# mkocabas/EpipolarPose

Measured on NVIDIA H100. Metric: multi-view samples/sec (4-view 256x256, bs32), higher is better.
Workload: dtype f16x3 (fp32 operands split into two fp16 planes, 3-pass error-compensated wgmma f16, f32 accumulate: fp32-grade results)

## Files before the change

epipolarpose_b200/_lib.py:

```python
import ctypes
import os

HERE = os.path.dirname(os.path.abspath(__file__))
LIB_PATH = os.environ.get("EPB_LIB_PATH") or os.path.join(HERE, "libepb.so")

EPB_MAX_TAPS = 64

c_int, c_i64, c_f, c_d, c_p = (ctypes.c_int, ctypes.c_int64, ctypes.c_float,
                               ctypes.c_double, ctypes.c_void_p)


class ConvGeom(ctypes.Structure):
    _fields_ = [("N", c_int), ("Hi", c_int), ("Wi", c_int), ("Cin", c_int),
                ("Ho", c_int), ("Wo", c_int), ("Cout", c_int),
                ("Hp", c_int), ("Wp", c_int),
                ("os", c_int), ("ph", c_int), ("pw", c_int), ("is_", c_int),
                ("T", c_int),
                ("dh", c_int * EPB_MAX_TAPS), ("dw", c_int * EPB_MAX_TAPS),
                ("wt", c_int * EPB_MAX_TAPS), ("Tw", c_int),
                ("in_relu", c_int), ("accumulate", c_int), ("precision", c_int)]


_PROTOS = {
    "epb_version": (c_int, []),
# ... 16 lines not shown
    "epb_bn_bwd_apply": (c_int, [c_p, c_p, c_p, c_p, c_p, c_p, c_p, c_p, c_int, c_p, c_i64, c_int, c_p, c_p, c_p, c_p]),
    "epb_add_masked": (c_int, [c_p, c_p, c_p, c_p, c_i64, c_p]),
    "epb_avgpool": (c_int, [c_p, c_p, c_int, c_int, c_int, c_p]),
    "epb_avgpool_bwd": (c_int, [c_p, c_p, c_int, c_int, c_int, c_int, c_p]),
    "epb_colsum": (c_int, [c_p, c_i64, c_int, c_p, c_p]),
    "epb_softargmax_fwd": (c_int, [c_p, c_int, c_int, c_int, c_int, c_int, c_int, c_p, c_p, c_p]),
    "epb_softargmax_bwd": (c_int, [c_p, c_int, c_int, c_int, c_int, c_int, c_int, c_p, c_p, c_p, c_p, c_p]),
    "epb_jointloss_fwd_bwd": (c_int, [c_p, c_p, c_p, c_int, c_int, c_int, c_f, c_p, c_p, c_p]),
    "epb_heatmap_joint_loss": (c_int, [c_p, c_p, c_p, c_int, c_int, c_f, c_p, c_p, c_p, c_int, c_int, c_f, c_f,
                                       c_p, c_p, c_p, c_p]),
    "epb_argmax2d": (c_int, [c_p, c_int, c_int, c_int, c_p, c_p, c_p, c_p]),
    "epb_final_preds": (c_int, [c_p, c_int, c_int, c_int, c_int, c_p, c_p, c_int, c_p, c_p, c_p]),
    "epb_patch_to_image": (c_int, [c_p, c_p, c_int, c_int, c_d, c_d, c_d, c_p, c_p]),
    "epb_triangulate": (c_int, [c_p, c_p, c_int, c_p, c_p, c_int, c_int, c_int, c_d, c_p, c_p, c_p]),
    "epb_triangulate_nview": (c_int, [c_p, c_int, c_p, c_int, c_int, c_int, c_p, c_p, c_p]),
    "epb_relative_pose": (c_int, [c_p, c_int, c_p, c_p, c_int, c_int, c_d, c_p, c_p, c_p, c_p, c_p, c_p,
                                  c_p]),
    "epb_project_labels": (c_int, [c_p, c_p, c_p, c_int, c_int, c_d, c_d, c_d, c_p, c_p, c_p]),
    "epb_h36m_eval": (c_int, [c_p, c_p, c_p, c_int, c_int, c_int, ctypes.c_uint32, c_d, c_p, c_p, c_p, c_p, c_p]),
    "epb_add3": (c_int, [c_p, c_p, c_p, c_p, c_i64, c_p]),
    "epb_mask_scale": (c_int, [c_p, c_p, c_f, c_p, c_i64, c_p]),
    "epb_patch_sample": (c_int, [c_p, c_p, c_p, c_p, c_p, c_p, c_p, c_int, c_int, c_int, c_p, c_p, c_p]),
    "epb_patch_sample_occ": (c_int, [c_p] * 7 + [c_int, c_int, c_int] + [c_p] * 5 + [c_p]),
    "epb_patch_joints": (c_int, [c_p, c_p, c_p, c_int, c_int, c_d, c_d, c_d, c_int, c_p, c_p]),
    "epb_bn_finalize_scale": (c_int, [c_p, c_i64, c_int, c_p, c_p, c_f, c_f] + [c_p] * 12),
    "epb_softargmax_bwd_split": (c_int, [c_p] + [c_int] * 5 + [c_p] * 7),
    "epb_act_scale": (c_int, [c_p, c_p, c_p, c_i64, c_int, c_p, c_p, c_p, c_p, c_p, c_p]),
    "epb_bn_act_split": (c_int, [c_p] * 8 + [c_int, c_i64, c_int, c_p, c_p, c_p, c_p]),
    "epb_bn_relu_maxpool_split": (c_int, [c_p] * 6 + [c_int] * 4 + [c_p]),
    "epb_im2col_split": (c_int, [c_p] * 3 + [c_int] * 11 + [c_p]),
    "epb_split16": (c_int, [c_p, ctypes.c_longlong, c_p, c_p, c_p, c_p]),
    "epb_split16_batch": (c_int, [c_p, c_int, ctypes.c_longlong, c_p, c_p]),
    "epb_conv16_fprop": (c_int, [ctypes.POINTER(ConvGeom)] + [c_p] * 8),
    "epb_conv16_wgrad": (c_int, [ctypes.POINTER(ConvGeom)] + [c_p] * 6 + [ctypes.c_longlong, c_p]),
    "epb_bn_bwd_reduce_mx": (c_int, [c_p] * 7 + [c_int, c_i64, c_int, c_p, c_p, c_p]),
    "epb_bn_bwd_apply_split": (c_int, [c_p] * 8 + [c_int, c_p, c_p, c_i64, c_int] + [c_p] * 6),
    "epb_bn_bwd_split": (c_int, [c_p] * 9 + [c_int, c_i64, c_int] + [c_p] * 6),
    "epb_avgpool_split": (c_int, [c_p, c_p, c_p, c_int, c_int, c_int, c_p]),
    "epb_sumsq": (c_int, [c_p, c_i64, c_p, c_p]),
    "epb_clip_scale": (c_int, [c_p, c_i64, c_p, c_d, c_p]),
    "epb_adam_step": (c_int, [c_p, c_p, c_p, c_p, c_i64, c_f, c_f, c_f, c_f, c_f, c_int, c_f, c_p]),
    "epb_sgd_step": (c_int, [c_p, c_p, c_p, c_i64, c_f, c_f, c_f, c_int, c_int, c_f, c_p]),
    "epb_adam_step_dev": (c_int, [c_p, c_p, c_p, c_p, c_i64, c_p, c_p, c_p]),
    "epb_sgd_step_dev": (c_int, [c_p, c_p, c_p, c_i64, c_p, c_p, c_p]),
}

EXPORTS = tuple(_PROTOS)


class EpbError(RuntimeError):
    pass


_lib = None


def lib():
    global _lib
    if _lib is None:
        if not os.path.exists(LIB_PATH):
            raise EpbError("libepb.so not built (%s); run `python -c 'import __graft_entry__ as g; "
                           "g.build()'`. There is no CPU fallback." % LIB_PATH)
        L = ctypes.CDLL(LIB_PATH)
        for name, (res, args) in _PROTOS.items():
            fn = getattr(L, name)
            fn.restype = res
            fn.argtypes = args
        _lib = L
    return _lib


def check(rc):
    if rc != 0:
        raise EpbError("libepb call failed (%d): %s" % (rc, lib().epb_last_error().decode()))


def call(name, *args):
    check(getattr(lib(), name)(*args))
```

epipolarpose_b200/csrc/conv16.cu:

```cuda
#include "split16_common.cuh"

namespace {

constexpr int BM = 128;
constexpr int kThreads16 = 384;
constexpr int kConsumers = 256;
constexpr int kStageBudget = 200 * 1024;
constexpr int kBoxBytes = 16 * 128;

struct Plan16 {
  epb_phase_grid grid;
  int Cout;
  int Wv, Hv;
  int T, CB;
  int n_tiles;
  int accumulate;
  int m_fastest;
  int koff[EPB_MAX_TAPS];
};

struct Maps16 {
  CUtensorMap a[4];
  CUtensorMap w;
  CUtensorMap out;
};

template <int BN>
struct Cfg16 {
  static constexpr int A_PLANE = BM * 128;
  static constexpr int B_PLANE = BN * 128;
  static constexpr int A_BYTES = 2 * A_PLANE;
  static constexpr int B_BYTES = 2 * B_PLANE;
  static constexpr int STAGE = A_BYTES + B_BYTES;
  static constexpr int S_ = kStageBudget / STAGE;
  static constexpr int S = S_ > 6 ? 6 : S_;
  static constexpr int BOX_BYTES = (kConsumers / 32) * kBoxBytes;
  static constexpr int STAT_BYTES = (kConsumers / 32) * 2 * BN * 4;
  static constexpr int SMEM =
      S * STAGE + BOX_BYTES + 1024  + 256  + STAT_BYTES;
  static_assert(SMEM <= 227 * 1024, "shared memory budget");
  static_assert(S >= 2, "ring too shallow");
};

template <int BN>
__global__ void __launch_bounds__(kThreads16, 1)
conv16_kernel(const __grid_constant__ Plan16 P, const __grid_constant__ Maps16 maps,
              const float* __restrict__ in_sc, const float* __restrict__ w_sc,
              const float* __restrict__ bias, double* __restrict__ stats) {
  using C = Cfg16<BN>;
  const epb_phase_grid& G = P.grid;
  constexpr int BOXES = C::S * C::STAGE;
  constexpr int CTRL = BOXES + C::BOX_BYTES;
  extern __shared__ uint8_t smem_raw[];
  tc::Ring<C::S, C::STAGE> ring(smem_raw, 0, CTRL, CTRL + 64);
  float* sstat = reinterpret_cast<float*>(ring.sm + CTRL + 256);

  const int warp = threadIdx.x >> 5, lane = threadIdx.x & 31;
  const int KB = P.T * P.CB;
  const int total_tiles = G.tiles * P.n_tiles;
  auto nt_of = [&](int tile) { return P.m_fastest ? tile / G.tiles : tile % P.n_tiles; };
  auto mt_of = [&](int tile) { return P.m_fastest ? tile % G.tiles : tile / P.n_tiles; };

  if (threadIdx.x == 0) ring.init(1, kConsumers / 32);
  __syncthreads();

  if (warp < 4) {
    if (warp == 0 && lane == 0) {
      for (int v = 0; v < 4; ++v) tc::tma_prefetch_desc(&maps.a[v]);
      tc::tma_prefetch_desc(&maps.w);
      tc::tma_prefetch_desc(&maps.out);
      for (int tile = blockIdx.x; tile < total_tiles; tile += gridDim.x) {
        const int nt = nt_of(tile);
        int w0, h0, n0;
        G.tile_origin(mt_of(tile), w0, h0, n0);
        int t = 0, cb = 0;
        for (int kb = 0; kb < KB; ++kb) {
          tc::mbar_wait(ring.empty(ring.stage), ring.phase ^ 1);
          const uint32_t fb = ring.full(ring.stage);
          tc::mbar_arrive_expect_tx(fb, C::STAGE);
          const uint32_t a_dst = ring.stage_addr(ring.stage);
          const CUtensorMap* am = &maps.a[G.map[t]];
          const int cx = cb * 64, wx = w0 + G.dwq[t], hx = h0 + G.dhq[t];
          tc::tma_load_5d(a_dst, am, fb, cx, wx, hx, n0, 0);
          tc::tma_load_5d(a_dst + C::A_PLANE, am, fb, cx, wx, hx, n0, 1);
          const uint32_t b_dst = a_dst + C::A_BYTES;
          const int kx = P.koff[t] + cx, rx = nt * BN;
          tc::tma_load_3d(b_dst, &maps.w, fb, kx, rx, 0);
          tc::tma_load_3d(b_dst + C::B_PLANE, &maps.w, fb, kx, rx, 1);
          if (++cb == P.CB) { cb = 0; ++t; }
          ring.advance();
        }
      }
    }
    return;
  }

  const int wgc = (warp >> 2) - 1;
  const int ct = threadIdx.x - 128;
  float* wstat = sstat + (ct >> 5) * 2 * BN;
  const int lc = (lane & 3) * 2;
  const int rb = wgc * 64 + (warp & 3) * 16;
  const int ra = rb + (lane >> 2);
  uint8_t* box = ring.sm + BOXES + (ct >> 5) * kBoxBytes;
  const uint32_t box_addr = tc::smem_u32(box);
  auto chunk = [&](int jj) { return ((2 * jj + ((lane & 3) >> 1)) ^ (lane >> 2)) * 16 + (lane & 1) * 8; };
  const float alpha = in_sc[1] * w_sc[1];
  const int twh = G.tw * G.th;
  if (stats) {
    for (int c = ct; c < (kConsumers / 32) * 2 * BN; c += kConsumers) sstat[c] = 0.f;
    tc::named_sync(1, kConsumers);
  }

  float acc[BN / 2];
  int nt_prev = -1;
  for (int tile = blockIdx.x; tile < total_tiles; tile += gridDim.x) {
    const int nt = nt_of(tile);
    if (stats && nt_prev >= 0 && nt != nt_prev)
      tc::stats_flush<BN, kConsumers / 32>(sstat, ct, nt_prev, P.Cout, stats);
    nt_prev = nt;
#pragma unroll
    for (int i = 0; i < BN / 2; ++i) acc[i] = 0.f;
    for (int kb = 0; kb < KB; ++kb)
      ring.consume(acc, [&](uint32_t st) {
        const uint32_t a_hi = st + wgc * 64 * 128, b_hi = st + C::A_BYTES;
#pragma unroll
        for (int kk = 0; kk < 4; ++kk)
          tc::mma3_f16<0, 0>(acc, tc::desc_kmajor_sw128(a_hi + kk * 32),
                             tc::desc_kmajor_sw128(a_hi + C::A_PLANE + kk * 32),
                             tc::desc_kmajor_sw128(b_hi + kk * 32),
                             tc::desc_kmajor_sw128(b_hi + C::B_PLANE + kk * 32));
      });
    ring.drain(acc);

    int w0, h0, n0;
    G.tile_origin(mt_of(tile), w0, h0, n0);
    bool srow[2];
#pragma unroll
    for (int h = 0; h < 2; ++h) {
      const int r = ra + 8 * h;
      const int w = w0 + r % G.tw, hh = h0 + (r / G.tw) % G.th, n = n0 + r / twh;
      srow[h] = w < G.Wp && hh < G.Hp && n < G.N;
    }
    const int bx = w0 + rb % G.tw, by = h0 + (rb / G.tw) % G.th, bz = n0 + rb / twh;
    const bool band = bx < P.Wv && by < P.Hv && bz < G.N;
#pragma unroll
    for (int q = 0; q < BN / 32; ++q) {
      if (lane == 0) tc::tma_store_wait_read<0>();
      __syncwarp();
#pragma unroll
      float v[4][2][2];
#pragma unroll
      for (int jj = 0; jj < 4; ++jj) {
        const int col = nt * BN + 32 * q + 8 * jj + lc;
        float2 b = make_float2(0.f, 0.f);
        if (bias && col < P.Cout) b = *reinterpret_cast<const float2*>(bias + col);
#pragma unroll
        for (int h = 0; h < 2; ++h) {
          v[jj][h][0] = acc[16 * q + 4 * jj + 2 * h] * alpha + b.x;
          v[jj][h][1] = acc[16 * q + 4 * jj + 2 * h + 1] * alpha + b.y;
          *reinterpret_cast<float2*>(box + 128 * ((lane >> 2) + 8 * h) + chunk(jj)) =
              make_float2(v[jj][h][0], v[jj][h][1]);
        }
      }
      tc::fence_proxy_async();
      __syncwarp();
      const int c0 = nt * BN + 32 * q;
      if (lane == 0 && band && c0 < P.Cout) {
        if (P.accumulate) tc::tma_reduce_add_4d(&maps.out, box_addr, c0, bx, by, bz);
        else tc::tma_store_4d(&maps.out, box_addr, c0, bx, by, bz);
        tc::tma_store_commit();
      }
      if (stats) {
#pragma unroll
        for (int jj = 0; jj < 4; ++jj) tc::stats_add<BN>(wstat, 32 * q + 8 * jj + lc, v[jj], srow);
      }
    }
  }
  if (stats && nt_prev >= 0) tc::stats_flush<BN, kConsumers / 32>(sstat, ct, nt_prev, P.Cout, stats);
  if (lane == 0) tc::tma_store_wait<0>();
}

}

extern "C" __attribute__((visibility("default"))) int epb_conv16_fprop(
    const epb_conv_geom* g, const epb_half* in, const float* in_sc, const epb_half* w,
    const float* w_sc, const float* bias, float* out, double* stats, epb_stream_t stream) {
  int rc = epb_conv_geom_check(g);
  if (rc) return rc;
  EPB_CHECK_ARG(in && in_sc && w && w_sc && out);
  EPB_CHECK_ARG(g->Cin % 64 == 0 && g->Cout % 4 == 0 && g->Cout >= 4);
  EPB_CHECK_ARG(g->is == 1 || g->is == 2);
  EPB_CHECK_ARG(!(stats && g->accumulate));
  EPB_CHECK_ARG((reinterpret_cast<uintptr_t>(in) & 127) == 0 && (reinterpret_cast<uintptr_t>(w) & 15) == 0);
  EPB_CHECK_ARG((reinterpret_cast<uintptr_t>(out) & 15) == 0 && (reinterpret_cast<uintptr_t>(bias) & 7) == 0);
  Plan16 P;
  Maps16 maps;
  memset(&maps, 0, sizeof(maps));
  bool dense;
  rc = epb_plan_phase_grid(g, in, BM, P.grid, maps.a, dense);
  if (rc) return rc;
  const int64_t Ho = dense ? 1 : g->Ho, Wo = dense ? P.grid.Wp : g->Wo, os = g->os;
  const int64_t ph = dense ? 0 : g->ph, pw = dense ? 0 : g->pw;
  P.Cout = g->Cout;
  P.Wv = dense ? P.grid.Wp : (g->Wo - g->pw + g->os - 1) / g->os;
  P.Hv = dense ? 1 : (g->Ho - g->ph + g->os - 1) / g->os;
  {
    const int bw = P.grid.tw < 16 ? P.grid.tw : 16;
    const int bh = P.grid.th < 16 / bw ? P.grid.th : 16 / bw;
    const int64_t C4 = (int64_t)g->Cout * 4;
    const cuuint64_t dims[4] = {(cuuint64_t)g->Cout, (cuuint64_t)P.Wv, (cuuint64_t)P.Hv,
                                (cuuint64_t)P.grid.N};
    const cuuint64_t strides[3] = {(cuuint64_t)(os * C4), (cuuint64_t)(os * Wo * C4),
                                   (cuuint64_t)(Ho * Wo * C4)};
    const cuuint32_t box[4] = {32, (cuuint32_t)bw, (cuuint32_t)bh, (cuuint32_t)(16 / (bw * bh))};
    rc = epb_encode_map(&maps.out, CU_TENSOR_MAP_DATA_TYPE_FLOAT32, 4, out + (ph * Wo + pw) * g->Cout,
                        dims, strides, box, CU_TENSOR_MAP_L2_PROMOTION_NONE, "output");
    if (rc) return rc;
  }
  P.T = g->T; P.CB = g->Cin / 64; P.accumulate = g->accumulate;
  for (int t = 0; t < g->T; ++t) P.koff[t] = g->wt[t] * g->Cin;
  P.m_fastest = stats != nullptr;
  const int bn = g->Cout <= 64 ? 64 : 128;
  P.n_tiles = (g->Cout + bn - 1) / bn;
  const int64_t K = (int64_t)g->Tw * g->Cin;
  const cuuint64_t dims[3] = {(cuuint64_t)K, (cuuint64_t)g->Cout, 2};
  const cuuint64_t strides[2] = {(cuuint64_t)K * 2, (cuuint64_t)K * 2 * g->Cout};
  const cuuint32_t box[3] = {64, (cuuint32_t)bn, 1};
  rc = epb_encode_map(&maps.w, CU_TENSOR_MAP_DATA_TYPE_FLOAT16, 3, w, dims, strides, box,
                      CU_TENSOR_MAP_L2_PROMOTION_L2_256B, "weights");
  if (rc) return rc;
  const int64_t tiles = (int64_t)P.grid.tiles * P.n_tiles;
  const unsigned grid = (unsigned)(tiles < kNumSMs ? tiles : kNumSMs);
  cudaStream_t st = as_stream(stream);
  if (bn == 64)
    return tc::launch<conv16_kernel<64>>(grid, kThreads16, Cfg16<64>::SMEM, st, P, maps, in_sc,
                                         w_sc, bias, stats);
  return tc::launch<conv16_kernel<128>>(grid, kThreads16, Cfg16<128>::SMEM, st, P, maps, in_sc,
                                        w_sc, bias, stats);
}
```

epipolarpose_b200/csrc/split16_common.cuh:

```cuda
#pragma once
#include "conv_common.cuh"
#include "tc_common.cuh"

typedef CUresult (*epb_encode_tiled_fn)(CUtensorMap*, CUtensorMapDataType, cuuint32_t, void*,
                                        const cuuint64_t*, const cuuint64_t*, const cuuint32_t*,
                                        const cuuint32_t*, CUtensorMapInterleave, CUtensorMapSwizzle,
                                        CUtensorMapL2promotion, CUtensorMapFloatOOBfill);
inline epb_encode_tiled_fn epb_get_encode_tiled() {
  static epb_encode_tiled_fn fn = nullptr;
  if (!fn) {
    void* p = nullptr;
    cudaDriverEntryPointQueryResult qr;
    if (cudaGetDriverEntryPoint("cuTensorMapEncodeTiled", &p, cudaEnableDefault, &qr) ==
            cudaSuccess && qr == cudaDriverEntryPointSuccess)
      fn = reinterpret_cast<epb_encode_tiled_fn>(p);
  }
  return fn;
}

inline int epb_encode_map(CUtensorMap* m, CUtensorMapDataType type, int rank, const void* base,
                          const cuuint64_t* dims, const cuuint64_t* strides, const cuuint32_t* box,
                          CUtensorMapL2promotion l2, const char* what) {
  epb_encode_tiled_fn enc = epb_get_encode_tiled();
  if (!enc) {
    epb_set_error("cuTensorMapEncodeTiled entry point unavailable");
    return EPB_ECUDA;
  }
  const cuuint32_t estr[5] = {1, 1, 1, 1, 1};
  const CUresult cr = enc(m, type, (cuuint32_t)rank, const_cast<void*>(base), dims, strides, box,
                          estr, CU_TENSOR_MAP_INTERLEAVE_NONE, CU_TENSOR_MAP_SWIZZLE_128B, l2,
                          CU_TENSOR_MAP_FLOAT_OOB_FILL_NONE);
  if (cr != CUDA_SUCCESS) {
    epb_set_error("cuTensorMapEncodeTiled(%s: dims %llu x %llu, box %u x %u) failed (%d)", what,
                  (unsigned long long)dims[0], (unsigned long long)dims[1], box[0], box[1], (int)cr);
    return EPB_ECUDA;
  }
  return EPB_OK;
}

inline void epb_choose_tile(int N, int Hp, int Wp, int rows, int& tw, int& th, int& tn) {
  long long best = -1;
  tw = rows; th = 1; tn = 1;
  for (int a = rows; a >= 1; a >>= 1) {
    for (int b = rows / a; b >= 1; b >>= 1) {
      const int c = rows / (a * b);
      const long long cov = (long long)((Wp + a - 1) / a) * ((Hp + b - 1) / b) * ((N + c - 1) / c);
      if (best < 0 || cov < best) { best = cov; tw = a; th = b; tn = c; }
    }
  }
}

inline int epb_make_act_map(CUtensorMap* m, const epb_half* base, int N, int H, int W, int C,
                            int stride, int qh, int qw, int tw, int th, int tn) {
  const int Wv = (W - qw + stride - 1) / stride, Hv = (H - qh + stride - 1) / stride;
  if (Wv <= 0 || Hv <= 0) {
    epb_set_error("empty strided view");
    return EPB_EINVAL;
  }
  const cuuint64_t dims[5] = {(cuuint64_t)C, (cuuint64_t)Wv, (cuuint64_t)Hv, (cuuint64_t)N, 2};
  const cuuint64_t strides[4] = {(cuuint64_t)stride * C * 2, (cuuint64_t)stride * W * C * 2,
                                 (cuuint64_t)H * W * C * 2, (cuuint64_t)N * H * W * C * 2};
  const cuuint32_t box[5] = {64, (cuuint32_t)tw, (cuuint32_t)th, (cuuint32_t)tn, 1};
  return epb_encode_map(m, CU_TENSOR_MAP_DATA_TYPE_FLOAT16, 5, base + ((int64_t)qh * W + qw) * C,
                        dims, strides, box, CU_TENSOR_MAP_L2_PROMOTION_L2_256B, "activation");
}

struct epb_phase_grid {
  int N, Hp, Wp;
  int tw, th, tn, tiles_w, tiles_h, tiles;
  short dwq[EPB_MAX_TAPS], dhq[EPB_MAX_TAPS];
  unsigned char map[EPB_MAX_TAPS];

  __host__ __device__ __forceinline__ void tile_origin(int it, int& w0, int& h0, int& n0) const {
    w0 = (it % tiles_w) * tw; it /= tiles_w;
    h0 = (it % tiles_h) * th;
    n0 = (it / tiles_h) * tn;
  }
};

inline int epb_plan_phase_grid(const epb_conv_geom* g, const epb_half* in, int rows,
                               epb_phase_grid& G, CUtensorMap (&maps)[4], bool& dense) {
  dense = g->T == 1 && g->is == 1 && g->os == 1 && g->dh[0] == 0 && g->dw[0] == 0 &&
          g->Hp == g->Hi && g->Wp == g->Wi && g->Hp == g->Ho && g->Wp == g->Wo;
  G.N = g->N; G.Hp = g->Hp; G.Wp = g->Wp;
  if (dense) {
    const int64_t M = (int64_t)g->N * g->Hp * g->Wp;
    EPB_CHECK_ARG(M < (1LL << 31));
    G.N = 1; G.Hp = 1; G.Wp = (int)M;
  }
  epb_choose_tile(G.N, G.Hp, G.Wp, rows, G.tw, G.th, G.tn);
  G.tiles_w = (G.Wp + G.tw - 1) / G.tw;
  G.tiles_h = (G.Hp + G.th - 1) / G.th;
  const int64_t tiles = (int64_t)G.tiles_w * G.tiles_h * ((G.N + G.tn - 1) / G.tn);
  EPB_CHECK_ARG(tiles < (1LL << 30));
  G.tiles = (int)tiles;
  bool need[4] = {false, false, false, false};
  for (int t = 0; t < g->T; ++t) {
    const int qh = ((g->dh[t] % g->is) + g->is) % g->is;
    const int qw = ((g->dw[t] % g->is) + g->is) % g->is;
    G.map[t] = (unsigned char)(qh * 2 + qw);
    G.dhq[t] = (short)((g->dh[t] - qh) / g->is);
    G.dwq[t] = (short)((g->dw[t] - qw) / g->is);
    need[qh * 2 + qw] = true;
  }
  const int Hi = dense ? 1 : g->Hi, Wi = dense ? G.Wp : g->Wi;
  for (int v = 0; v < 4; ++v) {
    if (!need[v]) continue;
    const int rc = epb_make_act_map(&maps[v], in, G.N, Hi, Wi, g->Cin, g->is, v >> 1, v & 1,
                                    G.tw, G.th, G.tn);
    if (rc) return rc;
  }
  for (int v = 0; v < 4; ++v)
    if (!need[v]) {
      for (int u = 0; u < 4; ++u)
        if (need[u]) { maps[v] = maps[u]; break; }
    }
  return EPB_OK;
}
```

epipolarpose_b200/csrc/tc_common.cuh:

```cuda
#pragma once
#include <cuda.h>
#include "common.cuh"

namespace tc {

__device__ __forceinline__ uint32_t smem_u32(const void* p) {
  return (uint32_t)__cvta_generic_to_shared(p);
}

__device__ __forceinline__ void mbar_init(uint32_t bar, uint32_t count) {
  asm volatile("mbarrier.init.shared::cta.b64 [%0], %1;" ::"r"(bar), "r"(count) : "memory");
}
__device__ __forceinline__ void fence_barrier_init() {
  asm volatile("fence.mbarrier_init.release.cluster;" ::: "memory");
}
__device__ __forceinline__ void mbar_arrive(uint32_t bar) {
  asm volatile("mbarrier.arrive.shared::cta.b64 _, [%0];" ::"r"(bar) : "memory");
}
__device__ __forceinline__ void mbar_arrive_expect_tx(uint32_t bar, uint32_t bytes) {
  asm volatile("mbarrier.arrive.expect_tx.shared::cta.b64 _, [%0], %1;" ::"r"(bar), "r"(bytes)
               : "memory");
}
__device__ __forceinline__ void mbar_wait(uint32_t bar, uint32_t parity) {
  uint32_t done = 0;
// ... 61 lines not shown
      "r"(src), "r"(c0), "r"(c1), "r"(c2), "r"(c3)
      : "memory");
}
__device__ __forceinline__ void tma_store_commit() {
  asm volatile("cp.async.bulk.commit_group;" ::: "memory");
}
template <int N>
__device__ __forceinline__ void tma_store_wait_read() {
  asm volatile("cp.async.bulk.wait_group.read %0;" ::"n"(N) : "memory");
}
template <int N>
__device__ __forceinline__ void tma_store_wait() {
  asm volatile("cp.async.bulk.wait_group %0;" ::"n"(N) : "memory");
}
__device__ __forceinline__ void tma_load_4d(uint32_t dst, const CUtensorMap* m, uint32_t bar,
                                            int c0, int c1, int c2, int c3) {
  asm volatile(
      "cp.async.bulk.tensor.4d.shared::cluster.global.mbarrier::complete_tx::bytes"
      " [%0], [%1, {%3, %4, %5, %6}], [%2];" ::"r"(dst), "l"(m), "r"(bar), "r"(c0), "r"(c1),
      "r"(c2), "r"(c3)
      : "memory");
}

__device__ __forceinline__ void wgmma_fence() {
  asm volatile("wgmma.fence.sync.aligned;" ::: "memory");
}
__device__ __forceinline__ void wgmma_commit() {
  asm volatile("wgmma.commit_group.sync.aligned;" ::: "memory");
}
template <int N>
__device__ __forceinline__ void wgmma_wait() {
  asm volatile("wgmma.wait_group.sync.aligned %0;" ::"n"(N) : "memory");
}
template <int R>
__device__ __forceinline__ void fence_acc(float (&d)[R]) {
#pragma unroll
  for (int i = 0; i < R; ++i) asm volatile("" : "+f"(d[i])::"memory");
}

__device__ __forceinline__ uint64_t desc_kmajor_sw128(uint32_t addr) {
  return (uint64_t)((addr & 0x3FFFF) >> 4) | ((uint64_t)1 << 16) | ((uint64_t)(1024 >> 4) << 32) |
         ((uint64_t)1 << 62);
}
__device__ __forceinline__ uint64_t desc_mnmajor16_sw128(uint32_t addr, uint32_t lbo_bytes,
                                                         uint32_t sbo_bytes) {
  return (uint64_t)((addr & 0x3FFFF) >> 4) | ((uint64_t)(lbo_bytes >> 4) << 16) |
         ((uint64_t)(sbo_bytes >> 4) << 32) | ((uint64_t)1 << 62);
}

#define EPB_ACC8(i) "+f"(d[i]), "+f"(d[i + 1]), "+f"(d[i + 2]), "+f"(d[i + 3]), \
                    "+f"(d[i + 4]), "+f"(d[i + 5]), "+f"(d[i + 6]), "+f"(d[i + 7])
template <int TA, int TB>
__device__ __forceinline__ void wgmma_f16_n64(float (&d)[32], uint64_t adesc, uint64_t bdesc,
                                                int scale_d) {
  asm volatile(
      "{\n\t.reg .pred p;\n\tsetp.ne.b32 p, %34, 0;\n\t"
      "wgmma.mma_async.sync.aligned.m64n64k16.f32.f16.f16 "
      "{%0, %1, %2, %3, %4, %5, %6, %7, %8, %9, %10, %11, %12, %13, %14, %15, %16, %17,"
      "%18, %19, %20, %21, %22, %23, %24, %25, %26, %27, %28, %29, %30, %31},"
      " %32, %33, p, 1, 1, %35, %36;\n\t}"
      : EPB_ACC8(0), EPB_ACC8(8), EPB_ACC8(16), EPB_ACC8(24)
      : "l"(adesc), "l"(bdesc), "r"(scale_d), "n"(TA), "n"(TB));
}

template <int TA, int TB>
__device__ __forceinline__ void wgmma_f16_n128(float (&d)[64], uint64_t adesc, uint64_t bdesc,
                                                int scale_d) {
  asm volatile(
      "{\n\t.reg .pred p;\n\tsetp.ne.b32 p, %66, 0;\n\t"
      "wgmma.mma_async.sync.aligned.m64n128k16.f32.f16.f16 "
      "{%0, %1, %2, %3, %4, %5, %6, %7, %8, %9, %10, %11, %12, %13, %14, %15, %16, %17,"
      "%18, %19, %20, %21, %22, %23, %24, %25, %26, %27, %28, %29, %30, %31, %32, %33, %34,"
      "%35, %36, %37, %38, %39, %40, %41, %42, %43, %44, %45, %46, %47, %48, %49, %50, %51,"
      "%52, %53, %54, %55, %56, %57, %58, %59, %60, %61, %62, %63},"
      " %64, %65, p, 1, 1, %67, %68;\n\t}"
      : EPB_ACC8(0), EPB_ACC8(8), EPB_ACC8(16), EPB_ACC8(24), EPB_ACC8(32), EPB_ACC8(40), EPB_ACC8(48), EPB_ACC8(56)
      : "l"(adesc), "l"(bdesc), "r"(scale_d), "n"(TA), "n"(TB));
}

__device__ __forceinline__ void wgmma_tf32_n32(float (&d)[16], uint64_t adesc, uint64_t bdesc,
                                                 int scale_d) {
  asm volatile(
      "{\n\t.reg .pred p;\n\tsetp.ne.b32 p, %18, 0;\n\t"
      "wgmma.mma_async.sync.aligned.m64n32k8.f32.tf32.tf32 "
      "{%0, %1, %2, %3, %4, %5, %6, %7, %8, %9, %10, %11, %12, %13, %14, %15},"
      " %16, %17, p, 1, 1;\n\t}"
      : EPB_ACC8(0), EPB_ACC8(8)
      : "l"(adesc), "l"(bdesc), "r"(scale_d));
}

__device__ __forceinline__ void wgmma_tf32_n64(float (&d)[32], uint64_t adesc, uint64_t bdesc,
                                                 int scale_d) {
  asm volatile(
      "{\n\t.reg .pred p;\n\tsetp.ne.b32 p, %34, 0;\n\t"
      "wgmma.mma_async.sync.aligned.m64n64k8.f32.tf32.tf32 "
      "{%0, %1, %2, %3, %4, %5, %6, %7, %8, %9, %10, %11, %12, %13, %14, %15, %16, %17,"
      "%18, %19, %20, %21, %22, %23, %24, %25, %26, %27, %28, %29, %30, %31},"
      " %32, %33, p, 1, 1;\n\t}"
      : EPB_ACC8(0), EPB_ACC8(8), EPB_ACC8(16), EPB_ACC8(24)
      : "l"(adesc), "l"(bdesc), "r"(scale_d));
}

__device__ __forceinline__ void wgmma_tf32_n128(float (&d)[64], uint64_t adesc, uint64_t bdesc,
                                                 int scale_d) {
  asm volatile(
      "{\n\t.reg .pred p;\n\tsetp.ne.b32 p, %66, 0;\n\t"
      "wgmma.mma_async.sync.aligned.m64n128k8.f32.tf32.tf32 "
      "{%0, %1, %2, %3, %4, %5, %6, %7, %8, %9, %10, %11, %12, %13, %14, %15, %16, %17,"
      "%18, %19, %20, %21, %22, %23, %24, %25, %26, %27, %28, %29, %30, %31, %32, %33, %34,"
      "%35, %36, %37, %38, %39, %40, %41, %42, %43, %44, %45, %46, %47, %48, %49, %50, %51,"
      "%52, %53, %54, %55, %56, %57, %58, %59, %60, %61, %62, %63},"
      " %64, %65, p, 1, 1;\n\t}"
      : EPB_ACC8(0), EPB_ACC8(8), EPB_ACC8(16), EPB_ACC8(24), EPB_ACC8(32), EPB_ACC8(40), EPB_ACC8(48), EPB_ACC8(56)
      : "l"(adesc), "l"(bdesc), "r"(scale_d));
}

template <int TA, int TB>
__device__ __forceinline__ void wgmma_f16(float (&d)[32], uint64_t a, uint64_t b, int sd) {
  wgmma_f16_n64<TA, TB>(d, a, b, sd);
}
template <int TA, int TB>
__device__ __forceinline__ void wgmma_f16(float (&d)[64], uint64_t a, uint64_t b, int sd) {
  wgmma_f16_n128<TA, TB>(d, a, b, sd);
}
__device__ __forceinline__ void wgmma_tf32(float (&d)[16], uint64_t a, uint64_t b, int sd) {
  wgmma_tf32_n32(d, a, b, sd);
}
__device__ __forceinline__ void wgmma_tf32(float (&d)[32], uint64_t a, uint64_t b, int sd) {
  wgmma_tf32_n64(d, a, b, sd);
}
__device__ __forceinline__ void wgmma_tf32(float (&d)[64], uint64_t a, uint64_t b, int sd) {
  wgmma_tf32_n128(d, a, b, sd);
}

template <int TA, int TB, int R>
__device__ __forceinline__ void mma3_f16(float (&d)[R], uint64_t ah, uint64_t al, uint64_t bh,
                                         uint64_t bl) {
  wgmma_f16<TA, TB>(d, al, bh, 1);
  wgmma_f16<TA, TB>(d, ah, bl, 1);
  wgmma_f16<TA, TB>(d, ah, bh, 1);
}
template <int R>
__device__ __forceinline__ void mma3_tf32(float (&d)[R], uint64_t ah, uint64_t al, uint64_t bh,
                                          uint64_t bl) {
  wgmma_tf32(d, al, bh, 1);
  wgmma_tf32(d, ah, bl, 1);
  wgmma_tf32(d, ah, bh, 1);
}

template <int S, int STAGE>
struct Ring {
  uint8_t* sm;
  uint32_t base, full0, empty0;
  int stage = 0, prev = -1;
  uint32_t phase = 0;

// ... 101 lines not shown
```

epipolarpose_b200/ops.py:

```python
import ctypes

import torch

from . import _lib
from ._lib import ConvGeom

launches = 0

_KERNELS_PER_CALL = {
    "epb_softargmax_fwd": 2, "epb_bn_bwd_apply": 2, "epb_colsum": 3,
    "epb_split16_batch": 3, "epb_split16": 3, "epb_bn_bwd_apply_split": 2, "epb_conv16_wgrad": 2,
    "epb_bn_bwd_reduce_mx": 2, "epb_bn_bwd_split": 3, "epb_softargmax_bwd_split": 3,
    "epb_patch_sample": 2, "epb_patch_sample_occ": 2,
}


def _stream():
    return ctypes.c_void_p(torch.cuda.current_stream().cuda_stream)


def _p(t, dtype=torch.float32):
    if t is None:
        return None
    if not t.is_cuda:
# ... 177 lines not shown


class SplitBatch:

    def __init__(self, jobs):
        import struct
        self.jobs = list(jobs)
        blob, first = b"", 0
        for (src, dst, sc) in self.jobs:
            n = src.numel()
            assert dst.numel() == 2 * n and dst.dtype == _H and sc.numel() == 2
            blob += struct.pack("<QQQqq", src.data_ptr(), dst.data_ptr(), sc.data_ptr(), n, first)
            first += (n + 2047) // 2048
        self.total_blocks = first
        dev = self.jobs[0][1].device
        self.table = torch.frombuffer(bytearray(blob), dtype=torch.uint8).to(dev)
        self.amax = torch.zeros(len(self.jobs), dtype=torch.int32, device=dev)


def split16(src, dst, sc, amax_ws):
    _call("epb_split16", _p(src), src.numel(), _p(dst, _H), _p(sc), _p(amax_ws, torch.int32), _stream())


def split16_batch(batch):
    _call("epb_split16_batch", _p(batch.table, torch.uint8), len(batch.jobs), batch.total_blocks,
          _p(batch.amax, torch.int32), _stream())


def conv16_fprop(g, x, x_sc, w, w_sc, out, bias=None, stats=None):
    _call("epb_conv16_fprop", ctypes.byref(g), _p(x, _H), _p(x_sc), _p(w, _H), _p(w_sc), _p(bias),
          _p(out), _p(stats, torch.float64), _stream())


def conv16_wgrad(g, x, x_sc, dout, dout_sc, dw, ws):
    _call("epb_conv16_wgrad", ctypes.byref(g), _p(x, _H), _p(x_sc), _p(dout, _H), _p(dout_sc),
          _p(dw), _p(ws), ws.numel() if ws is not None else 0, _stream())


def bn_bwd_reduce_mx(dy, x, mask_hi, scale, shift, mean, invstd, relu, M, C, sums, maxes):
    _call("epb_bn_bwd_reduce_mx", _p(dy), _p(x), _p(mask_hi, _H), _p(scale), _p(shift), _p(mean),
          _p(invstd), int(relu), M, C, _p(sums, torch.float64), _p(maxes), _stream())


def bn_bwd_apply_split(dy, x, mask_hi, scale, shift, mean, invstd, gamma, relu, sums, maxes, M, C,
                       dz, dz_sc, dy_masked, dgamma, dbeta):
    _call("epb_bn_bwd_apply_split", _p(dy), _p(x), _p(mask_hi, _H), _p(scale), _p(shift), _p(mean),
          _p(invstd), _p(gamma), int(relu), _p(sums, torch.float64), _p(maxes), M, C, _p(dz, _H),
          _p(dz_sc), _p(dy_masked), _p(dgamma), _p(dbeta), _stream())


def bn_bwd_split(dy, x, mask_hi, scale, shift, mean, invstd, gamma, relu, M, C, dz, dz_sc, dy_masked,
                 dgamma, dbeta, mask_bits=None):
    _call("epb_bn_bwd_split", _p(dy), _p(x), _p(mask_hi, _H), _p(mask_bits, torch.uint8), _p(scale),
          _p(shift), _p(mean),
          _p(invstd), _p(gamma), int(relu), M, C, _p(dz, _H), _p(dz_sc), _p(dy_masked), _p(dgamma),
          _p(dbeta), _stream())


def avgpool_split(x, x_sc, y, N, HW, C):
    _call("epb_avgpool_split", _p(x, _H), _p(x_sc), _p(y), N, HW, C, _stream())



def softargmax_fwd(logits, layout, N, J, D, H, W, coords, lse):
    _call("epb_softargmax_fwd", _p(logits), layout, N, J, D, H, W, _p(coords), _p(lse), _stream())

# ... 131 lines not shown
```

include/epb.h:

```cpp
#ifndef EPB_H_
#define EPB_H_

#include <stdint.h>

#ifdef __cplusplus
extern "C" {
#endif

#define EPB_OK 0
#define EPB_EINVAL (-1)
#define EPB_ECUDA (-2)
#define EPB_ENOGPU (-3)

#define EPB_MAX_TAPS 64

typedef void* epb_stream_t;

int epb_version(void);
const char* epb_last_error(void);
int epb_device_check(void);

typedef struct {
  int N, Hi, Wi, Cin;
  int Ho, Wo, Cout;
// ... 85 lines not shown
                  const float* res_sc, float* sc, epb_stream_t stream);
int epb_bn_finalize_scale(const double* stats, int64_t M, int C, const float* gamma,
                          const float* beta, float eps, float momentum, float* running_mean,
                          float* running_var, float* scale, float* shift, float* mean,
                          float* invstd, const double* stats2, const float* scale2,
                          const float* shift2, const float* res_sc, float* sc, epb_stream_t stream);
int epb_bn_act_split(const float* x, const float* scale, const float* shift,
                     const float* r, const float* rscale, const float* rshift,
                     const epb_half* r_split, const float* r_sc, int relu,
                     int64_t M, int C, epb_half* y, const float* y_sc,
                     uint8_t* mask_bits, epb_stream_t stream);
int epb_bn_relu_maxpool_split(const float* x, const float* scale, const float* shift,
                              epb_half* y, const float* y_sc, uint8_t* argidx, int N,
                              int H, int W, int C, epb_stream_t stream);
int epb_im2col_split(const float* img_nchw, epb_half* col, const float* col_sc, int N,
                     int C, int Hi, int Wi, int kh, int kw, int stride, int pad, int Ho,
                     int Wo, int Kpad, epb_stream_t stream);
typedef struct epb_split_job {
  const float* src;
  epb_half* dst;
  float* sc;
  long long n;
  long long first_block;
} epb_split_job;
int epb_split16_batch(const epb_split_job* jobs, int njobs, long long total_blocks,
                      uint32_t* amax_ws, epb_stream_t stream);

int epb_split16(const float* src, long long n, epb_half* dst, float* sc, uint32_t* amax_ws,
                epb_stream_t stream);

int epb_conv16_fprop(const epb_conv_geom* g, const epb_half* in, const float* in_sc,
                     const epb_half* w, const float* w_sc, const float* bias,
                     float* out, double* stats, epb_stream_t stream);
int epb_conv16_wgrad(const epb_conv_geom* g, const epb_half* in, const float* in_sc,
                     const epb_half* dout, const float* dout_sc, float* dw, float* ws,
                     long long ws_floats, epb_stream_t stream);

int epb_bn_bwd_reduce_mx(const float* dy, const float* x, const epb_half* mask_hi,
                         const float* scale, const float* shift, const float* mean,
                         const float* invstd, int relu, int64_t M, int C, double* sums,
                         float* maxes, epb_stream_t stream);
int epb_bn_bwd_apply_split(const float* dy, const float* x, const epb_half* mask_hi,
                           const float* scale, const float* shift, const float* mean,
                           const float* invstd, const float* gamma, int relu,
                           const double* sums, const float* maxes, int64_t M, int C,
                           epb_half* dz, float* dz_sc, float* dy_masked, float* dgamma,
                           float* dbeta, epb_stream_t stream);
int epb_bn_bwd_split(const float* dy, const float* x, const epb_half* mask_hi,
                     const uint8_t* mask_bits, const float* scale, const float* shift, const float* mean, const float* invstd,
                     const float* gamma, int relu, int64_t M, int C, epb_half* dz, float* dz_sc,
                     float* dy_masked, float* dgamma, float* dbeta, epb_stream_t stream);
int epb_avgpool_split(const epb_half* x, const float* x_sc, float* y, int N, int HW, int C,
                      epb_stream_t stream);

int epb_softargmax_fwd(const float* logits, int layout, int N, int J, int D,
                       int H, int W, float* coords, float* lse_ws,
                       epb_stream_t stream);
int epb_softargmax_bwd(const float* logits, int layout, int N, int J, int D,
                       int H, int W, const float* coords, const float* lse_ws,
                       const float* dcoords, float* dlogits,
                       epb_stream_t stream);
int epb_softargmax_bwd_split(const float* logits, int N, int J, int D, int H, int W,
                             const float* coords, const float* lse_ws, const float* dcoords,
                             epb_half* dlogits16, float* sc, float* dbias, epb_stream_t stream);

int epb_jointloss_fwd_bwd(const float* x, const float* t, const float* w, int n,
// ... 76 lines not shown
```

Baseline: 486.9.

## Add 256-wide output tile path for split-f16 conv forward with register rebalancing

Adds a BN=256 variant of the warp-specialized wgmma conv kernel that uses m64n256k16 instructions, a 32-channel K chunk with 64B swizzle so the stage fits in shared memory, and setmaxnreg to move registers from producer warps to the consumer warpgroups. A heuristic chooses the wide tile for large Cout layers that have enough tiles to fill the SMs, with an environment override. The aim is more reuse of each A tile across output channels and fewer tile loads. The cost is higher register pressure, halved K per stage (more barrier round-trips), and possible wave quantization on some layers.

```diff
diff --git a/epipolarpose_b200/_lib.py b/epipolarpose_b200/_lib.py
--- a/epipolarpose_b200/_lib.py
+++ b/epipolarpose_b200/_lib.py
@@ -72,6 +72,7 @@
     "epb_split16": (c_int, [c_p, ctypes.c_longlong, c_p, c_p, c_p, c_p]),
     "epb_split16_batch": (c_int, [c_p, c_int, ctypes.c_longlong, c_p, c_p]),
     "epb_conv16_fprop": (c_int, [ctypes.POINTER(ConvGeom)] + [c_p] * 8),
+    "epb_conv16_set_tile_width": (c_int, [c_int]),
     "epb_conv16_wgrad": (c_int, [ctypes.POINTER(ConvGeom)] + [c_p] * 6 + [ctypes.c_longlong, c_p]),
     "epb_bn_bwd_reduce_mx": (c_int, [c_p] * 7 + [c_int, c_i64, c_int, c_p, c_p, c_p]),
     "epb_bn_bwd_apply_split": (c_int, [c_p] * 8 + [c_int, c_p, c_p, c_i64, c_int] + [c_p] * 6),
@@ -107,6 +108,9 @@
             fn.restype = res
             fn.argtypes = args
         _lib = L
+        bn = os.environ.get("EPB_CONV16_BN")
+        if bn:
+            check(L.epb_conv16_set_tile_width(int(bn)))
     return _lib
 
 
diff --git a/epipolarpose_b200/csrc/conv16.cu b/epipolarpose_b200/csrc/conv16.cu
--- a/epipolarpose_b200/csrc/conv16.cu
+++ b/epipolarpose_b200/csrc/conv16.cu
@@ -27,8 +27,9 @@
 
 template <int BN>
 struct Cfg16 {
-  static constexpr int A_PLANE = BM * 128;
-  static constexpr int B_PLANE = BN * 128;
+  static constexpr int KC = BN == 256 ? 32 : 64;
+  static constexpr int A_PLANE = BM * KC * 2;
+  static constexpr int B_PLANE = BN * KC * 2;
   static constexpr int A_BYTES = 2 * A_PLANE;
   static constexpr int B_BYTES = 2 * B_PLANE;
   static constexpr int STAGE = A_BYTES + B_BYTES;
@@ -64,7 +65,9 @@
   if (threadIdx.x == 0) ring.init(1, kConsumers / 32);
   __syncthreads();
 
+  constexpr bool kMoveRegs = BN == 256;
   if (warp < 4) {
+    if constexpr (kMoveRegs) tc::setmaxnreg_dec<40>();
     if (warp == 0 && lane == 0) {
       for (int v = 0; v < 4; ++v) tc::tma_prefetch_desc(&maps.a[v]);
       tc::tma_prefetch_desc(&maps.w);
@@ -80,7 +83,7 @@
           tc::mbar_arrive_expect_tx(fb, C::STAGE);
           const uint32_t a_dst = ring.stage_addr(ring.stage);
           const CUtensorMap* am = &maps.a[G.map[t]];
-          const int cx = cb * 64, wx = w0 + G.dwq[t], hx = h0 + G.dhq[t];
+          const int cx = cb * C::KC, wx = w0 + G.dwq[t], hx = h0 + G.dhq[t];
           tc::tma_load_5d(a_dst, am, fb, cx, wx, hx, n0, 0);
           tc::tma_load_5d(a_dst + C::A_PLANE, am, fb, cx, wx, hx, n0, 1);
           const uint32_t b_dst = a_dst + C::A_BYTES;
@@ -95,6 +98,7 @@
     return;
   }
 
+  if constexpr (kMoveRegs) tc::setmaxnreg_inc<232>();
   const int wgc = (warp >> 2) - 1;
   const int ct = threadIdx.x - 128;
   float* wstat = sstat + (ct >> 5) * 2 * BN;
@@ -122,13 +126,14 @@
     for (int i = 0; i < BN / 2; ++i) acc[i] = 0.f;
     for (int kb = 0; kb < KB; ++kb)
       ring.consume(acc, [&](uint32_t st) {
-        const uint32_t a_hi = st + wgc * 64 * 128, b_hi = st + C::A_BYTES;
-#pragma unroll
-        for (int kk = 0; kk < 4; ++kk)
-          tc::mma3_f16<0, 0>(acc, tc::desc_kmajor_sw128(a_hi + kk * 32),
-                             tc::desc_kmajor_sw128(a_hi + C::A_PLANE + kk * 32),
-                             tc::desc_kmajor_sw128(b_hi + kk * 32),
-                             tc::desc_kmajor_sw128(b_hi + C::B_PLANE + kk * 32));
+        const uint32_t a_hi = st + wgc * 64 * C::KC * 2, b_hi = st + C::A_BYTES;
+        auto desc = [](uint32_t a) {
+          return C::KC == 64 ? tc::desc_kmajor_sw128(a) : tc::desc_kmajor_sw64(a);
+        };
+#pragma unroll
+        for (int kk = 0; kk < C::KC / 16; ++kk)
+          tc::mma3_f16<0, 0>(acc, desc(a_hi + kk * 32), desc(a_hi + C::A_PLANE + kk * 32),
+                             desc(b_hi + kk * 32), desc(b_hi + C::B_PLANE + kk * 32));
       });
     ring.drain(acc);
 
@@ -147,7 +152,6 @@
     for (int q = 0; q < BN / 32; ++q) {
       if (lane == 0) tc::tma_store_wait_read<0>();
       __syncwarp();
-#pragma unroll
       float v[4][2][2];
 #pragma unroll
       for (int jj = 0; jj < 4; ++jj) {
@@ -180,6 +184,25 @@
   if (lane == 0) tc::tma_store_wait<0>();
 }
 
+int g_tile_width = 0;
+
+int tile_width(const epb_conv_geom* g, int64_t m_tiles) {
+  if (g->Cout <= 64) return 64;
+  if (g_tile_width) return g_tile_width;
+  const int64_t pad128 = (g->Cout + 127) / 128 * 128 - g->Cout;
+  const int64_t pad256 = (g->Cout + 255) / 256 * 256 - g->Cout;
+  const bool wide = g->Cout >= 256 && m_tiles * ((g->Cout + 255) / 256) >= kNumSMs &&
+                    pad256 <= pad128 && !g->accumulate && !(g->is == 2 && g->T == 16) &&
+                    !(g->os == 2 && g->T <= 2);
+  return wide ? 256 : 128;
+}
+
+}
+
+extern "C" __attribute__((visibility("default"))) int epb_conv16_set_tile_width(int bn) {
+  EPB_CHECK_ARG(bn == 0 || bn == 128 || bn == 256);
+  g_tile_width = bn;
+  return EPB_OK;
 }
 
 extern "C" __attribute__((visibility("default"))) int epb_conv16_fprop(
@@ -199,6 +222,12 @@
   bool dense;
   rc = epb_plan_phase_grid(g, in, BM, P.grid, maps.a, dense);
   if (rc) return rc;
+  const int bn = tile_width(g, P.grid.tiles);
+  const int kc = bn == 256 ? Cfg16<256>::KC : 64;
+  if (kc != 64) {
+    rc = epb_plan_phase_grid(g, in, BM, P.grid, maps.a, dense, kc);
+    if (rc) return rc;
+  }
   const int64_t Ho = dense ? 1 : g->Ho, Wo = dense ? P.grid.Wp : g->Wo, os = g->os;
   const int64_t ph = dense ? 0 : g->ph, pw = dense ? 0 : g->pw;
   P.Cout = g->Cout;
@@ -217,17 +246,16 @@
                         dims, strides, box, CU_TENSOR_MAP_L2_PROMOTION_NONE, "output");
     if (rc) return rc;
   }
-  P.T = g->T; P.CB = g->Cin / 64; P.accumulate = g->accumulate;
+  P.T = g->T; P.CB = g->Cin / kc; P.accumulate = g->accumulate;
   for (int t = 0; t < g->T; ++t) P.koff[t] = g->wt[t] * g->Cin;
   P.m_fastest = stats != nullptr;
-  const int bn = g->Cout <= 64 ? 64 : 128;
   P.n_tiles = (g->Cout + bn - 1) / bn;
   const int64_t K = (int64_t)g->Tw * g->Cin;
   const cuuint64_t dims[3] = {(cuuint64_t)K, (cuuint64_t)g->Cout, 2};
   const cuuint64_t strides[2] = {(cuuint64_t)K * 2, (cuuint64_t)K * 2 * g->Cout};
-  const cuuint32_t box[3] = {64, (cuuint32_t)bn, 1};
+  const cuuint32_t box[3] = {(cuuint32_t)kc, (cuuint32_t)bn, 1};
   rc = epb_encode_map(&maps.w, CU_TENSOR_MAP_DATA_TYPE_FLOAT16, 3, w, dims, strides, box,
-                      CU_TENSOR_MAP_L2_PROMOTION_L2_256B, "weights");
+                      CU_TENSOR_MAP_L2_PROMOTION_L2_256B, "weights", epb_kblock_swizzle(kc));
   if (rc) return rc;
   const int64_t tiles = (int64_t)P.grid.tiles * P.n_tiles;
   const unsigned grid = (unsigned)(tiles < kNumSMs ? tiles : kNumSMs);
@@ -235,6 +263,9 @@
   if (bn == 64)
     return tc::launch<conv16_kernel<64>>(grid, kThreads16, Cfg16<64>::SMEM, st, P, maps, in_sc,
                                          w_sc, bias, stats);
+  if (bn == 256)
+    return tc::launch<conv16_kernel<256>>(grid, kThreads16, Cfg16<256>::SMEM, st, P, maps, in_sc,
+                                          w_sc, bias, stats);
   return tc::launch<conv16_kernel<128>>(grid, kThreads16, Cfg16<128>::SMEM, st, P, maps, in_sc,
                                         w_sc, bias, stats);
 }
diff --git a/epipolarpose_b200/csrc/split16_common.cuh b/epipolarpose_b200/csrc/split16_common.cuh
--- a/epipolarpose_b200/csrc/split16_common.cuh
+++ b/epipolarpose_b200/csrc/split16_common.cuh
@@ -20,7 +20,8 @@
 
 inline int epb_encode_map(CUtensorMap* m, CUtensorMapDataType type, int rank, const void* base,
                           const cuuint64_t* dims, const cuuint64_t* strides, const cuuint32_t* box,
-                          CUtensorMapL2promotion l2, const char* what) {
+                          CUtensorMapL2promotion l2, const char* what,
+                          CUtensorMapSwizzle swizzle = CU_TENSOR_MAP_SWIZZLE_128B) {
   epb_encode_tiled_fn enc = epb_get_encode_tiled();
   if (!enc) {
     epb_set_error("cuTensorMapEncodeTiled entry point unavailable");
@@ -28,7 +29,7 @@
   }
   const cuuint32_t estr[5] = {1, 1, 1, 1, 1};
   const CUresult cr = enc(m, type, (cuuint32_t)rank, const_cast<void*>(base), dims, strides, box,
-                          estr, CU_TENSOR_MAP_INTERLEAVE_NONE, CU_TENSOR_MAP_SWIZZLE_128B, l2,
+                          estr, CU_TENSOR_MAP_INTERLEAVE_NONE, swizzle, l2,
                           CU_TENSOR_MAP_FLOAT_OOB_FILL_NONE);
   if (cr != CUDA_SUCCESS) {
     epb_set_error("cuTensorMapEncodeTiled(%s: dims %llu x %llu, box %u x %u) failed (%d)", what,
@@ -50,8 +51,11 @@
   }
 }
 
+inline CUtensorMapSwizzle epb_kblock_swizzle(int kc) {
+  return kc == 32 ? CU_TENSOR_MAP_SWIZZLE_64B : CU_TENSOR_MAP_SWIZZLE_128B;
+}
 inline int epb_make_act_map(CUtensorMap* m, const epb_half* base, int N, int H, int W, int C,
-                            int stride, int qh, int qw, int tw, int th, int tn) {
+                            int stride, int qh, int qw, int tw, int th, int tn, int kc = 64) {
   const int Wv = (W - qw + stride - 1) / stride, Hv = (H - qh + stride - 1) / stride;
   if (Wv <= 0 || Hv <= 0) {
     epb_set_error("empty strided view");
@@ -60,9 +64,10 @@
   const cuuint64_t dims[5] = {(cuuint64_t)C, (cuuint64_t)Wv, (cuuint64_t)Hv, (cuuint64_t)N, 2};
   const cuuint64_t strides[4] = {(cuuint64_t)stride * C * 2, (cuuint64_t)stride * W * C * 2,
                                  (cuuint64_t)H * W * C * 2, (cuuint64_t)N * H * W * C * 2};
-  const cuuint32_t box[5] = {64, (cuuint32_t)tw, (cuuint32_t)th, (cuuint32_t)tn, 1};
+  const cuuint32_t box[5] = {(cuuint32_t)kc, (cuuint32_t)tw, (cuuint32_t)th, (cuuint32_t)tn, 1};
   return epb_encode_map(m, CU_TENSOR_MAP_DATA_TYPE_FLOAT16, 5, base + ((int64_t)qh * W + qw) * C,
-                        dims, strides, box, CU_TENSOR_MAP_L2_PROMOTION_L2_256B, "activation");
+                        dims, strides, box, CU_TENSOR_MAP_L2_PROMOTION_L2_256B, "activation",
+                        epb_kblock_swizzle(kc));
 }
 
 struct epb_phase_grid {
@@ -79,7 +84,8 @@
 };
 
 inline int epb_plan_phase_grid(const epb_conv_geom* g, const epb_half* in, int rows,
-                               epb_phase_grid& G, CUtensorMap (&maps)[4], bool& dense) {
+                               epb_phase_grid& G, CUtensorMap (&maps)[4], bool& dense,
+                               int kc = 64) {
   dense = g->T == 1 && g->is == 1 && g->os == 1 && g->dh[0] == 0 && g->dw[0] == 0 &&
           g->Hp == g->Hi && g->Wp == g->Wi && g->Hp == g->Ho && g->Wp == g->Wo;
   G.N = g->N; G.Hp = g->Hp; G.Wp = g->Wp;
@@ -107,7 +113,7 @@
   for (int v = 0; v < 4; ++v) {
     if (!need[v]) continue;
     const int rc = epb_make_act_map(&maps[v], in, G.N, Hi, Wi, g->Cin, g->is, v >> 1, v & 1,
-                                    G.tw, G.th, G.tn);
+                                    G.tw, G.th, G.tn, kc);
     if (rc) return rc;
   }
   for (int v = 0; v < 4; ++v)
diff --git a/epipolarpose_b200/csrc/tc_common.cuh b/epipolarpose_b200/csrc/tc_common.cuh
--- a/epipolarpose_b200/csrc/tc_common.cuh
+++ b/epipolarpose_b200/csrc/tc_common.cuh
@@ -117,6 +117,14 @@
 __device__ __forceinline__ void wgmma_wait() {
   asm volatile("wgmma.wait_group.sync.aligned %0;" ::"n"(N) : "memory");
 }
+template <int N>
+__device__ __forceinline__ void setmaxnreg_dec() {
+  asm volatile("setmaxnreg.dec.sync.aligned.u32 %0;" ::"n"(N));
+}
+template <int N>
+__device__ __forceinline__ void setmaxnreg_inc() {
+  asm volatile("setmaxnreg.inc.sync.aligned.u32 %0;" ::"n"(N));
+}
 template <int R>
 __device__ __forceinline__ void fence_acc(float (&d)[R]) {
 #pragma unroll
@@ -126,6 +134,10 @@
 __device__ __forceinline__ uint64_t desc_kmajor_sw128(uint32_t addr) {
   return (uint64_t)((addr & 0x3FFFF) >> 4) | ((uint64_t)1 << 16) | ((uint64_t)(1024 >> 4) << 32) |
          ((uint64_t)1 << 62);
+}
+__device__ __forceinline__ uint64_t desc_kmajor_sw64(uint32_t addr) {
+  return (uint64_t)((addr & 0x3FFFF) >> 4) | ((uint64_t)1 << 16) | ((uint64_t)(512 >> 4) << 32) |
+         ((uint64_t)2 << 62);
 }
 __device__ __forceinline__ uint64_t desc_mnmajor16_sw128(uint32_t addr, uint32_t lbo_bytes,
                                                          uint32_t sbo_bytes) {
@@ -163,6 +175,27 @@
       : "l"(adesc), "l"(bdesc), "r"(scale_d), "n"(TA), "n"(TB));
 }
 
+template <int TA, int TB>
+__device__ __forceinline__ void wgmma_f16_n256(float (&d)[128], uint64_t adesc, uint64_t bdesc,
+                                                int scale_d) {
+  asm volatile(
+      "{\n\t.reg .pred p;\n\tsetp.ne.b32 p, %130, 0;\n\t"
+      "wgmma.mma_async.sync.aligned.m64n256k16.f32.f16.f16 "
+      "{%0, %1, %2, %3, %4, %5, %6, %7, %8, %9, %10, %11, %12, %13, %14, %15, %16, %17,"
+      "%18, %19, %20, %21, %22, %23, %24, %25, %26, %27, %28, %29, %30, %31, %32, %33, %34,"
+      "%35, %36, %37, %38, %39, %40, %41, %42, %43, %44, %45, %46, %47, %48, %49, %50, %51,"
+      "%52, %53, %54, %55, %56, %57, %58, %59, %60, %61, %62, %63, %64, %65, %66, %67, %68,"
+      "%69, %70, %71, %72, %73, %74, %75, %76, %77, %78, %79, %80, %81, %82, %83, %84, %85,"
+      "%86, %87, %88, %89, %90, %91, %92, %93, %94, %95, %96, %97, %98, %99, %100, %101,"
+      "%102, %103, %104, %105, %106, %107, %108, %109, %110, %111, %112, %113, %114, %115,"
+      "%116, %117, %118, %119, %120, %121, %122, %123, %124, %125, %126, %127},"
+      " %128, %129, p, 1, 1, %131, %132;\n\t}"
+      : EPB_ACC8(0), EPB_ACC8(8), EPB_ACC8(16), EPB_ACC8(24), EPB_ACC8(32), EPB_ACC8(40), EPB_ACC8(48), EPB_ACC8(56),
+        EPB_ACC8(64), EPB_ACC8(72), EPB_ACC8(80), EPB_ACC8(88), EPB_ACC8(96), EPB_ACC8(104), EPB_ACC8(112),
+        EPB_ACC8(120)
+      : "l"(adesc), "l"(bdesc), "r"(scale_d), "n"(TA), "n"(TB));
+}
+
 __device__ __forceinline__ void wgmma_tf32_n32(float (&d)[16], uint64_t adesc, uint64_t bdesc,
                                                  int scale_d) {
   asm volatile(
@@ -207,6 +240,10 @@
 template <int TA, int TB>
 __device__ __forceinline__ void wgmma_f16(float (&d)[64], uint64_t a, uint64_t b, int sd) {
   wgmma_f16_n128<TA, TB>(d, a, b, sd);
+}
+template <int TA, int TB>
+__device__ __forceinline__ void wgmma_f16(float (&d)[128], uint64_t a, uint64_t b, int sd) {
+  wgmma_f16_n256<TA, TB>(d, a, b, sd);
 }
 __device__ __forceinline__ void wgmma_tf32(float (&d)[16], uint64_t a, uint64_t b, int sd) {
   wgmma_tf32_n32(d, a, b, sd);
diff --git a/epipolarpose_b200/ops.py b/epipolarpose_b200/ops.py
--- a/epipolarpose_b200/ops.py
+++ b/epipolarpose_b200/ops.py
@@ -233,6 +233,10 @@
           _p(out), _p(stats, torch.float64), _stream())
 
 
+def conv16_set_tile_width(bn):
+    _lib.call("epb_conv16_set_tile_width", int(bn))
+
+
 def conv16_wgrad(g, x, x_sc, dout, dout_sc, dw, ws):
     _call("epb_conv16_wgrad", ctypes.byref(g), _p(x, _H), _p(x_sc), _p(dout, _H), _p(dout_sc),
           _p(dw), _p(ws), ws.numel() if ws is not None else 0, _stream())
diff --git a/include/epb.h b/include/epb.h
--- a/include/epb.h
+++ b/include/epb.h
@@ -141,6 +141,7 @@
 int epb_conv16_fprop(const epb_conv_geom* g, const epb_half* in, const float* in_sc,
                      const epb_half* w, const float* w_sc, const float* bias,
                      float* out, double* stats, epb_stream_t stream);
+int epb_conv16_set_tile_width(int bn);
 int epb_conv16_wgrad(const epb_conv_geom* g, const epb_half* in, const float* in_sc,
                      const epb_half* dout, const float* dout_sc, float* dw, float* ws,
                      long long ws_floats, epb_stream_t stream);
```

Result: faster. 495.4, median of 6 (+1.7%).
